# nerfstudio-project/nerfstudio

Hardware: AMD Instinct MI355X
Metric: training rays/sec (4096 rays x 48 samples per GPU) (higher is better)
Workload: dtype f32

## Files before the change

### nerfstudio_amd/csrc/density_mlp.hip

```cpp
#include "common.h"
#include "density_point.h"
#include "proposal_chain.h"

namespace nsamd {

constexpr int kMlpBlock = 256;
constexpr int kMaxBlocks = 768;
constexpr int kDensityActMax = 2048;

__host__ __device__ constexpr int density_partial_stride(int in_dim, int hidden) {
  return (hidden * in_dim + 2 * hidden + 1 + 3) & ~3;
}

template <int IN, int H>
__global__ __launch_bounds__(kMlpBlock) void density_mlp_fwd_kernel(const float* __restrict__ enc,
                                                                    const float* __restrict__ selector, int64_t M,
                                                                    nsamd_density_mlp mlp,
                                                                    float* __restrict__ density,
                                                                    float* __restrict__ pre_out) {
  const float* __restrict__ W0 = mlp.W0;
  const float* __restrict__ b0 = mlp.b0;
  const float* __restrict__ W1 = mlp.W1;
  for (int64_t p = (int64_t)blockIdx.x * kMlpBlock + threadIdx.x; p < M; p += (int64_t)gridDim.x * kMlpBlock) {
    float x[IN];
#pragma unroll
    for (int k = 0; k < IN; ++k) x[k] = enc[(int64_t)k * M + p];
    float out = mlp.b1[0];
    constexpr int JU = (H <= 16) ? H : 4;
#pragma unroll JU
    for (int j = 0; j < H; ++j) {
      float a = b0[j];
#pragma unroll
      for (int k = 0; k < IN; ++k) a = fmaf(W0[j * IN + k], x[k], a);
      out = fmaf(W1[j], fmaxf(a, 0.0f), out);
    }
    const float sel = selector ? selector[p] : 1.0f;
    if (pre_out) pre_out[p] = out;
    density[p] = mlp.average_init_density * expf(out) * sel;
  }
}

template <int LEVELS, int H>
__global__ __launch_bounds__(kMlpBlock) void density_field_fwd_kernel(nsamd_points P, int64_t M, int transform,
                                                                      nsamd_aabb box, const float2* __restrict__ table,
                                                                      nsamd_grid grid, nsamd_density_mlp mlp,
                                                                      float* __restrict__ enc_out,
                                                                      float* __restrict__ selector_out,
                                                                      float* __restrict__ density,
                                                                      float* __restrict__ pre_out) {
  const int64_t p = (int64_t)blockIdx.x * kMlpBlock + threadIdx.x;
  if (p >= M) return;
  float x, y, z;
  load_position(P, p, x, y, z);
  density_point<LEVELS, H>(x, y, z, p, M, transform, box, table, grid, mlp, enc_out, selector_out, density, pre_out);
// ... 179 lines not shown
    float* row = partials + (size_t)blockIdx.x * density_partial_stride(IN, H);
    for (int e = threadIdx.x; e < H * IN; e += kMlpBlock) row[e] = red[(e / IN) * 16 + (e % IN)];
    if (threadIdx.x < 2 * H + 1) row[H * IN + threadIdx.x] = accV;
    return;
  }
  for (int e = threadIdx.x; e < H * IN; e += kMlpBlock) unsafeAtomicAdd(dW0 + e, red[(e / IN) * 16 + (e % IN)]);
  if (threadIdx.x < H) unsafeAtomicAdd(db0 + threadIdx.x, accV);
  else if (threadIdx.x < 2 * H) unsafeAtomicAdd(dW1 + (threadIdx.x - H), accV);
  else if (threadIdx.x == 2 * H) unsafeAtomicAdd(db1, accV);
}

template <int IN, int H>
__global__ __launch_bounds__(kMlpBlock) void density_mlp_bwd_kernel(
    const float* __restrict__ enc, const float* __restrict__ selector, const float* __restrict__ pre,
    const float* __restrict__ ddensity, int64_t M, nsamd_density_mlp mlp, float* __restrict__ denc,
    float* __restrict__ dW0, float* __restrict__ db0, float* __restrict__ dW1, float* __restrict__ db1,
    float* __restrict__ partials, const uint32_t* __restrict__ gate, const uint8_t* __restrict__ ray_mask, int spr) {
  density_mlp_bwd_body<IN, H>(enc, selector, pre, ddensity, M, mlp, denc, dW0, db0, dW1, db1, partials, gate, ray_mask, spr,
                              (int)gridDim.x);
}

struct DensityBwdArgs {
  const float* enc;
  const float* selector;
  const float* pre;
  const float* ddensity;
  int64_t M;
  nsamd_density_mlp mlp;
  float* denc;
  float* dW0;
  float* db0;
  float* dW1;
  float* db1;
  float* partials;
  const uint32_t* gate;
  const uint8_t* ray_mask;
  int spr;
  int nblocks;
};

template <int IN, int H>
__global__ __launch_bounds__(kMlpBlock) void density_mlp_bwd_pair_kernel(DensityBwdArgs a, DensityBwdArgs b) {
  if (blockIdx.y == 0) {
    if ((int)blockIdx.x >= a.nblocks) return;
    density_mlp_bwd_body<IN, H>(a.enc, a.selector, a.pre, a.ddensity, a.M, a.mlp, a.denc, a.dW0, a.db0, a.dW1, a.db1,
                                a.partials, a.gate, a.ray_mask, a.spr, a.nblocks);
  } else {
    if ((int)blockIdx.x >= b.nblocks) return;
    density_mlp_bwd_body<IN, H>(b.enc, b.selector, b.pre, b.ddensity, b.M, b.mlp, b.denc, b.dW0, b.db0, b.dW1, b.db1,
                                b.partials, b.gate, b.ray_mask, b.spr, b.nblocks);
  }
}

constexpr int kDwGroups = 16;
__device__ __forceinline__ void density_dw_reduce_body(const float* __restrict__ partials, int rows, int stride, int n_w0,
                                                       int hidden, float* __restrict__ dW0, float* __restrict__ db0,
                                                       float* __restrict__ dW1, float* __restrict__ db1,
                                                       const uint32_t* __restrict__ gate) {
  if (gate != nullptr && __hip_atomic_load(gate, __ATOMIC_RELAXED, __HIP_MEMORY_SCOPE_AGENT) == 0u) return;
  __shared__ float part[kDwGroups][64];
  const int el = threadIdx.x & 63, grp = threadIdx.x >> 6;
  const int e = blockIdx.x * 64 + el;
  const int total = n_w0 + 2 * hidden + 1;
  float s = 0.f;
  if (e < total) {
    for (int b0i = grp; b0i < rows; b0i += kDwGroups * 16) {
      float v[16];
#pragma unroll
      for (int u = 0; u < 16; ++u) {
        const int b = b0i + u * kDwGroups;
        v[u] = partials[(size_t)(b < rows ? b : rows - 1) * stride + e];
      }
#pragma unroll
      for (int u = 0; u < 16; ++u) s += (b0i + u * kDwGroups < rows) ? v[u] : 0.0f;
    }
  }
  part[grp][el] = s;
  __syncthreads();
  if (grp == 0 && e < total) {
    float t = 0.f;
#pragma unroll
    for (int g2 = 0; g2 < kDwGroups; ++g2) t += part[g2][el];
    float* dst = e < n_w0 ? dW0 + e : (e < n_w0 + hidden ? db0 + (e - n_w0) : (e < n_w0 + 2 * hidden ? dW1 + (e - n_w0 - hidden) : db1));
    *dst += t;
  }
}

__global__ __launch_bounds__(64 * kDwGroups) void density_dw_reduce_kernel(const float* __restrict__ partials, int rows,
                                                                            int stride, int n_w0, int hidden,
                                                                            float* __restrict__ dW0,
                                                                            float* __restrict__ db0,
                                                                            float* __restrict__ dW1,
                                                                            float* __restrict__ db1,
                                                                            const uint32_t* __restrict__ gate) {
  density_dw_reduce_body(partials, rows, stride, n_w0, hidden, dW0, db0, dW1, db1, gate);
}

__global__ __launch_bounds__(64 * kDwGroups) void density_dw_reduce_pair_kernel(DensityBwdArgs a, DensityBwdArgs b, int stride,
                                                                                 int n_w0, int hidden) {
  if (blockIdx.y == 0) density_dw_reduce_body(a.partials, a.nblocks, stride, n_w0, hidden, a.dW0, a.db0, a.dW1, a.db1, a.gate);
  else density_dw_reduce_body(b.partials, b.nblocks, stride, n_w0, hidden, b.dW0, b.db0, b.dW1, b.db1, b.gate);
}

template <int IN, int H>
static int launch_fwd(const float* enc, const float* selector, int64_t M, nsamd_density_mlp mlp, float* density,
                      float* pre, hipStream_t stream) {
  const unsigned blocks = (unsigned)min((int64_t)8192, (M + kMlpBlock - 1) / kMlpBlock);
  density_mlp_fwd_kernel<IN, H><<<blocks, kMlpBlock, 0, stream>>>(enc, selector, M, mlp, density, pre);
  NSAMD_CHECK_LAUNCH();
  return NSAMD_OK;
}

template <int IN, int H>
static int launch_bwd(const float* enc, const float* selector, const float* pre, const float* ddensity, int64_t M,
                      nsamd_density_mlp mlp, float* denc, float* dW0, float* db0, float* dW1, float* db1,
                      float* workspace, int64_t workspace_floats, const uint32_t* gate, const uint8_t* ray_mask, int spr,
                      hipStream_t stream) {
  const unsigned blocks = (unsigned)min((int64_t)kMaxBlocks, (M + kMlpBlock - 1) / kMlpBlock);
  const size_t lds = sizeof(float) * ((size_t)(2 * H + IN + 1) * (kMlpBlock + 1) + 8 + (size_t)H * (((IN + 3) & ~3) + 2)) +
                     kDensityActMax;
  if (lds > 64 * 1024) {
    if (hipFuncSetAttribute(reinterpret_cast<const void*>(&density_mlp_bwd_kernel<IN, H>),
                            hipFuncAttributeMaxDynamicSharedMemorySize, (int)lds) != hipSuccess)
      return NSAMD_ERR_LAUNCH;
  }
  constexpr int stride = density_partial_stride(IN, H);
  float* partials = (workspace != nullptr && workspace_floats >= (int64_t)blocks * stride) ? workspace : nullptr;
  density_mlp_bwd_kernel<IN, H><<<blocks, kMlpBlock, lds, stream>>>(enc, selector, pre, ddensity, M, mlp, denc, dW0,
                                                                   db0, dW1, db1, partials, gate, ray_mask, spr);
  NSAMD_CHECK_LAUNCH();
  if (partials != nullptr) {
    const int total = H * IN + 2 * H + 1;
    density_dw_reduce_kernel<<<(total + 63) / 64, 64 * kDwGroups, 0, stream>>>(partials, (int)blocks, stride, H * IN, H,
                                                                             dW0, db0, dW1, db1, gate);
    NSAMD_CHECK_LAUNCH();
  }
  return NSAMD_OK;
}

template <int IN, int H>
static int launch_bwd_pair(const DensityBwdCall& a, const DensityBwdCall& b, hipStream_t stream) {
  const DensityBwdCall* c[2] = {&a, &b};
  const size_t lds = sizeof(float) * ((size_t)(2 * H + IN + 1) * (kMlpBlock + 1) + 8 + (size_t)H * (((IN + 3) & ~3) + 2)) +
                     kDensityActMax;
  if (lds > 64 * 1024) {
    if (hipFuncSetAttribute(reinterpret_cast<const void*>(&density_mlp_bwd_pair_kernel<IN, H>),
                            hipFuncAttributeMaxDynamicSharedMemorySize, (int)lds) != hipSuccess)
      return NSAMD_ERR_LAUNCH;
  }
  constexpr int stride = density_partial_stride(IN, H);
  DensityBwdArgs k[2];
  unsigned gx = 0;
  for (int i = 0; i < 2; ++i) {
    const unsigned blocks = (unsigned)min((int64_t)kMaxBlocks, (c[i]->M + kMlpBlock - 1) / kMlpBlock);
    if (c[i]->workspace == nullptr || c[i]->workspace_floats < (int64_t)blocks * stride) return NSAMD_ERR_UNSUPPORTED;
    k[i] = DensityBwdArgs{c[i]->enc, c[i]->selector, c[i]->pre, c[i]->ddensity, c[i]->M, c[i]->mlp, c[i]->denc, c[i]->dW0,
                          c[i]->db0, c[i]->dW1, c[i]->db1, c[i]->workspace, c[i]->gate, c[i]->ray_mask,
                          c[i]->ray_mask ? c[i]->spr : 1, (int)blocks};
    gx = blocks > gx ? blocks : gx;
  }
  if (a.workspace == b.workspace || a.dW0 == b.dW0) return NSAMD_ERR_UNSUPPORTED;
  density_mlp_bwd_pair_kernel<IN, H><<<dim3(gx, 2u), kMlpBlock, lds, stream>>>(k[0], k[1]);
  NSAMD_CHECK_LAUNCH();
  const int total = H * IN + 2 * H + 1;
  density_dw_reduce_pair_kernel<<<dim3((total + 63) / 64, 2u), 64 * kDwGroups, 0, stream>>>(k[0], k[1], stride, H * IN, H);
  NSAMD_CHECK_LAUNCH();
  return NSAMD_OK;
}

int density_bwd_launch_pair(const DensityBwdCall& a, const DensityBwdCall& b, hipStream_t stream) {
  if (a.mlp.in_dim != b.mlp.in_dim || a.mlp.hidden != b.mlp.hidden || a.M <= 0 || b.M <= 0) return NSAMD_ERR_UNSUPPORTED;
  if (a.mlp.in_dim == 10 && a.mlp.hidden == 16) return launch_bwd_pair<10, 16>(a, b, stream);
  if (a.mlp.in_dim == 16 && a.mlp.hidden == 16) return launch_bwd_pair<16, 16>(a, b, stream);
  if (a.mlp.in_dim == 10 && a.mlp.hidden == 64) return launch_bwd_pair<10, 64>(a, b, stream);
  if (a.mlp.in_dim == 16 && a.mlp.hidden == 64) return launch_bwd_pair<16, 64>(a, b, stream);
  return NSAMD_ERR_UNSUPPORTED;
}

}

using namespace nsamd;

#define NSAMD_DENSITY_DISPATCH(CALL)                                  \
  if (mlp.in_dim == 10 && mlp.hidden == 16) return CALL(10, 16);      \
  if (mlp.in_dim == 16 && mlp.hidden == 16) return CALL(16, 16);      \
  if (mlp.in_dim == 10 && mlp.hidden == 64) return CALL(10, 64);      \
  if (mlp.in_dim == 16 && mlp.hidden == 64) return CALL(16, 64);      \
  return NSAMD_ERR_UNSUPPORTED;

extern "C" int nsamd_density_mlp_fwd(const float* enc, const float* selector, int64_t M, nsamd_density_mlp mlp,
                                     float* density, float* pre, nsamd_stream_t stream) {
  NSAMD_REQUIRE(M >= 0);
  if (M == 0) return NSAMD_OK;
  NSAMD_REQUIRE(enc && density && mlp.W0 && mlp.b0 && mlp.W1 && mlp.b1);
#define CALL(IN, H) launch_fwd<IN, H>(enc, selector, M, mlp, density, pre, (hipStream_t)stream)
  NSAMD_DENSITY_DISPATCH(CALL)
#undef CALL
}

extern "C" int nsamd_density_field_fwd(nsamd_points pts, int64_t M, int transform, nsamd_aabb aabb, const float* table,
                                       nsamd_grid grid, nsamd_density_mlp mlp, float* enc, float* selector, float* density,
                                       float* pre, nsamd_stream_t stream) {
  NSAMD_REQUIRE(M >= 0);
  if (M == 0) return NSAMD_OK;
  NSAMD_REQUIRE(table && density && mlp.W0 && mlp.b0 && mlp.W1 && mlp.b1);
  NSAMD_REQUIRE(transform >= 0 && transform <= 2);
  if (pts.positions == nullptr) {
    NSAMD_REQUIRE(pts.origins && pts.directions && pts.t_bins && pts.samples_per_ray > 0 && M % pts.samples_per_ray == 0);
  }
  if (grid.log2_table_size < 1 || grid.log2_table_size > 28) return NSAMD_ERR_UNSUPPORTED;
  if (mlp.in_dim != 2 * grid.num_levels) return NSAMD_ERR_INVALID_ARG;
  const int64_t nb = (M + kMlpBlock - 1) / kMlpBlock;
  if (nb > 0x7fffffffLL) return NSAMD_ERR_UNSUPPORTED;
  const float2* t2 = reinterpret_cast<const float2*>(table);
#define NSAMD_DENSITY_FWD(L_, H_)                                                                                       \
  density_field_fwd_kernel<L_, H_><<<(unsigned)nb, kMlpBlock, 0, (hipStream_t)stream>>>(pts, M, transform, aabb, t2, grid, mlp, \
                                                                                      enc, selector, density, pre)
  if (grid.num_levels == 5 && mlp.hidden == 16) {
    NSAMD_DENSITY_FWD(5, 16);
  } else if (grid.num_levels == 8 && mlp.hidden == 16) {
    NSAMD_DENSITY_FWD(8, 16);
  } else if (grid.num_levels == 5 && mlp.hidden == 64) {
    NSAMD_DENSITY_FWD(5, 64);
  } else if (grid.num_levels == 8 && mlp.hidden == 64) {
    NSAMD_DENSITY_FWD(8, 64);
  } else {
    return NSAMD_ERR_UNSUPPORTED;
  }
// ... 35 lines not shown
```

### nerfstudio_amd/csrc/proposal_chain.h

```cpp
#pragma once

#include "common.h"

namespace nsamd {

struct WeightsBwdCall {
  const float* t_bins;
  const float* density;
  const float* dweights;
  int64_t num_rays;
  int32_t S;
  float* ddensity;
  uint32_t* gate;
  uint8_t* ray_mask;
};
int weights_bwd_launch_pair(const WeightsBwdCall& a, const WeightsBwdCall& b, hipStream_t stream);

struct DensityBwdCall {
  const float* enc;
  const float* selector;
  const float* pre;
  const float* ddensity;
  int64_t M;
  nsamd_density_mlp mlp;
  float* denc;
  float* dW0;
  float* db0;
  float* dW1;
  float* db1;
  float* workspace;
  int64_t workspace_floats;
  const uint32_t* gate;
  const uint8_t* ray_mask;
  int spr;
};
int density_bwd_launch_pair(const DensityBwdCall& a, const DensityBwdCall& b, hipStream_t stream);

}
```

### nerfstudio_amd/csrc/proposal_chain.hip

```cpp
#include "proposal_chain.h"
#include "scatter.h"

using namespace nsamd;

static int level_checks(const nsamd_proposal_level_bwd& l) {
  NSAMD_REQUIRE(l.num_rays > 0 && l.samples_per_ray > 0 && l.samples_per_ray <= 1024);
  NSAMD_REQUIRE(l.t_bins && l.density && l.dweights && l.ddensity && l.gate && l.ray_mask);
  NSAMD_REQUIRE(l.enc && l.pre && l.denc && l.dW0 && l.db0 && l.dW1 && l.db1 && l.mlp.W0 && l.mlp.b0 && l.mlp.W1 && l.mlp.b1);
  NSAMD_REQUIRE(l.origins && l.directions && l.table && l.dtable && l.scatter_workspace);
  NSAMD_REQUIRE(l.transform >= 0 && l.transform <= 2);
  NSAMD_REQUIRE(l.grid.num_levels > 0 && l.grid.num_levels <= NSAMD_MAX_LEVELS && 2 * l.grid.num_levels == l.mlp.in_dim);
  if (l.grid.log2_table_size < 1 || l.grid.log2_table_size > 28) return NSAMD_ERR_UNSUPPORTED;
  return NSAMD_OK;
}

static nsamd_points level_points(const nsamd_proposal_level_bwd& l) {
  nsamd_points p{};
  p.positions = nullptr;
  p.origins = l.origins;
  p.directions = l.directions;
  p.t_bins = l.t_bins;
  p.samples_per_ray = l.samples_per_ray;
  return p;
}

static int weights_single(const nsamd_proposal_level_bwd& l, nsamd_stream_t st) {
  return nsamd_weights_bwd_gate(l.t_bins, l.density, l.dweights, l.num_rays, l.samples_per_ray, l.ddensity, l.gate, l.ray_mask,
                                1, st);
}
static int density_single(const nsamd_proposal_level_bwd& l, nsamd_stream_t st) {
  return nsamd_density_mlp_bwd_gated(l.enc, l.selector, l.pre, l.ddensity, l.num_rays * l.samples_per_ray, l.mlp, l.denc, l.dW0,
                                     l.db0, l.dW1, l.db1, l.mlp_workspace, l.mlp_workspace_floats, l.gate, l.ray_mask,
                                     l.samples_per_ray, st);
}
static int scatter_single(const nsamd_proposal_level_bwd& l, nsamd_stream_t st) {
  const int64_t M = l.num_rays * l.samples_per_ray;
  return nsamd_hashgrid_encode_bwd_gated(level_points(l), M, l.transform, l.aabb, l.table, l.grid, l.denc, 1, M, l.dtable,
                                         l.scatter_workspace, l.scatter_workspace_floats, l.gate, l.ray_mask, st);
}

extern "C" int nsamd_proposal_levels_bwd(const nsamd_proposal_level_bwd* levels, int32_t num_levels, int32_t gates_precleared,
                                         nsamd_stream_t stream) {
  NSAMD_REQUIRE(num_levels >= 0 && (num_levels == 0 || levels != nullptr));
  hipStream_t st = (hipStream_t)stream;
  for (int i = 0; i < num_levels; ++i) {
    const int rc = level_checks(levels[i]);
    if (rc) return rc;
  }
  if (!gates_precleared) {
    for (int i = 0; i < num_levels; ++i)
      if (hipMemsetAsync(levels[i].gate, 0, sizeof(uint32_t), st) != hipSuccess) return NSAMD_ERR_LAUNCH;
  }
  for (int i = 0; i < num_levels; i += 2) {
    const nsamd_proposal_level_bwd& a = levels[i];
    if (i + 1 >= num_levels) {
      int rc = weights_single(a, stream);
      if (!rc) rc = density_single(a, stream);
      if (!rc) rc = scatter_single(a, stream);
      if (rc) return rc;
      break;
    }
    const nsamd_proposal_level_bwd& b = levels[i + 1];
    const int64_t Ma = a.num_rays * a.samples_per_ray, Mb = b.num_rays * b.samples_per_ray;
    int rc = weights_bwd_launch_pair(
        WeightsBwdCall{a.t_bins, a.density, a.dweights, a.num_rays, a.samples_per_ray, a.ddensity, a.gate, a.ray_mask},
        WeightsBwdCall{b.t_bins, b.density, b.dweights, b.num_rays, b.samples_per_ray, b.ddensity, b.gate, b.ray_mask}, st);
    if (rc == NSAMD_ERR_UNSUPPORTED) {
      rc = weights_single(a, stream);
      if (!rc) rc = weights_single(b, stream);
    }
    if (rc) return rc;
    rc = density_bwd_launch_pair(
        DensityBwdCall{a.enc, a.selector, a.pre, a.ddensity, Ma, a.mlp, a.denc, a.dW0, a.db0, a.dW1, a.db1, a.mlp_workspace,
                       a.mlp_workspace_floats, a.gate, a.ray_mask, a.samples_per_ray},
        DensityBwdCall{b.enc, b.selector, b.pre, b.ddensity, Mb, b.mlp, b.denc, b.dW0, b.db0, b.dW1, b.db1, b.mlp_workspace,
                       b.mlp_workspace_floats, b.gate, b.ray_mask, b.samples_per_ray},
        st);
    if (rc == NSAMD_ERR_UNSUPPORTED) {
      rc = density_single(a, stream);
      if (!rc) rc = density_single(b, stream);
    }
    if (rc) return rc;
    ScatterPlan pa = scatter_plan(a.grid, Ma, false), pb = scatter_plan(b.grid, Mb, false);
    rc = NSAMD_ERR_UNSUPPORTED;
    if (pa.ok && pb.ok && pa.total_words <= a.scatter_workspace_floats && pb.total_words <= b.scatter_workspace_floats) {
      rc = scatter_launch_pair(
          ScatterCall{level_points(a), Ma, a.transform, a.aabb, a.grid, a.denc, 1, Ma, a.dtable, a.scatter_workspace, pa, false,
                      a.gate, a.ray_mask},
          ScatterCall{level_points(b), Mb, b.transform, b.aabb, b.grid, b.denc, 1, Mb, b.dtable, b.scatter_workspace, pb, false,
                      b.gate, b.ray_mask},
          st);
    }
    if (rc == NSAMD_ERR_UNSUPPORTED) {
      rc = scatter_single(a, stream);
      if (!rc) rc = scatter_single(b, stream);
    }
    if (rc) return rc;
  }
  return NSAMD_OK;
}
```

### nerfstudio_amd/csrc/scatter.h

```cpp
#pragma once

#include "common.h"

namespace nsamd {

struct FixedScale {
  int k;
  bool empty;
  bool bad;
};

__device__ __forceinline__ FixedScale fixed_scale(uint32_t max_bits, int headroom) {
  FixedScale s;
  const int e_max = (int)((max_bits >> 23) & 0xffu);
  s.empty = e_max == 0;
  s.bad = e_max == 255;
  s.k = 188 - headroom - e_max;
  return s;
}

#ifndef NSAMD_FIXED_ROUND
#define NSAMD_FIXED_ROUND 0
#endif
__device__ __forceinline__ unsigned long long to_fixed(float v, int k) {
// ... 99 lines not shown
    float* a = t + 2 * (size_t)(rec.w & 0x3fffu);
    unsafeAtomicAdd(a, f0);
    unsafeAtomicAdd(a + 1, f1);
  }
  atomicAdd(hdr + kHdrEvtUnordered, 1u);
}

__device__ __forceinline__ void spill_append(const ScatterBufs& buf, uint32_t cap, uint32_t tile, const uint4& rec) {
  if (spill_list_append(buf.hdr, buf.spill_rec, buf.spill_tile, cap, tile, rec)) return;
  if (buf.direct_table != nullptr) {
    const uint32_t level = tile >> buf.log2_bins, bin = tile & ((1u << buf.log2_bins) - 1u);
    spill_direct(buf.direct_table + ((((size_t)level << buf.log2_table_size) + ((size_t)bin << buf.slice_log2)) << 1),
                 buf.hdr, rec);
  } else {
    atomicAdd(buf.hdr + kHdrEvtLost, 1u);
  }
}

struct PairHash {
  uint32_t ia, ib;
};

__device__ __forceinline__ PairHash pair_hash(const Cell& c, int q, uint32_t mask) {
  const uint32_t yz = ((uint32_t)((q & 1) ? c.hi[1] : c.lo[1]) * kPrimeY) ^ ((uint32_t)((q & 2) ? c.hi[2] : c.lo[2]) * kPrimeZ);
  return PairHash{((uint32_t)c.lo[0] ^ yz) & mask, ((uint32_t)c.hi[0] ^ yz) & mask};
}

#endif

struct ScatterPlan {
  bool ok;
  ScatterGeom geom;
  int64_t tiles;
  int64_t state_words;
  int64_t total_words;
};

ScatterPlan scatter_plan(const nsamd_grid& grid, int64_t M, bool max_spill);

ScatterPlan scatter_plan_producers(const nsamd_grid& grid, int64_t M, int workgroups, int seg_cap);

ScatterBufs scatter_bufs(float* workspace, const ScatterPlan& p);

struct ReduceRider;
bool scatter_apply_takes_rider(const ScatterPlan& plan);
int scatter_apply_launch(const nsamd_grid& grid, const ScatterPlan& plan, float* workspace, float* dtable, bool overwrite,
                         hipStream_t stream, const ReduceRider* rider = nullptr);

int scatter_launch(const nsamd_points& pts, int64_t M, int transform, const nsamd_aabb& aabb, const nsamd_grid& grid,
                   const float* denc, int64_t stride_p, int64_t stride_k, float* dtable, float* workspace,
                   const ScatterPlan& plan, bool overwrite, const uint32_t* gate, const uint8_t* ray_mask,
                   hipStream_t stream);

struct ScatterCall {
  nsamd_points pts;
  int64_t M;
  int transform;
  nsamd_aabb aabb;
  nsamd_grid grid;
  const float* denc;
  int64_t stride_p, stride_k;
  float* dtable;
  float* workspace;
  ScatterPlan plan;
  bool overwrite;
  const uint32_t* gate;
  const uint8_t* ray_mask;
};
int scatter_launch_pair(const ScatterCall& a, const ScatterCall& b, hipStream_t stream);

}
```

### nerfstudio_amd/csrc/scatter.hip

```cpp

#include <type_traits>

#include "field_reduce.h"
#include "scatter.h"

NSAMD_PROBE_DEFINE(scatter)

namespace nsamd {

__device__ __forceinline__ bool gate_is_clear(const uint32_t* gate) {
  return gate != nullptr && __hip_atomic_load(gate, __ATOMIC_RELAXED, __HIP_MEMORY_SCOPE_AGENT) == 0u;
}

constexpr int kRunLen = 4;
constexpr int kRunThreads = 256;
constexpr int kMaxLog2Bins = 10;

template <int kThreads, int kPts, int kLevels>
__global__ __launch_bounds__(kThreads) void scatter_route_fine_kernel(
    nsamd_points P, int64_t M, int transform, nsamd_aabb box, nsamd_grid grid, const float* __restrict__ denc,
    int64_t stride_p, int64_t stride_k, ScatterGeom G, LevelList levels, ScatterBufs buf,
    const uint32_t* __restrict__ gate, const uint8_t* __restrict__ ray_mask) {
  static_assert(kPts * kLevels * 4 <= 32, "overflow mask is 32 bits");
  if (gate_is_clear(gate)) return;
  extern __shared__ __attribute__((aligned(16))) uint32_t lds_u[];
  const int B = 1 << G.log2_bins;
  uint32_t* cnt = lds_u;
  uint32_t* cnt2 = cnt + kLevels * B;
  uint32_t* base = cnt2 + kLevels * B;
  uint32_t* lmax = base + kLevels * B;
  PROBE_STAMP(0, 0);
  for (int t = threadIdx.x; t < 2 * kLevels * B; t += kThreads) cnt[t] = 0u;
  if (threadIdx.x < kLevels) lmax[threadIdx.x] = 0u;
  const int first = blockIdx.y * kLevels;
  int lvl[kLevels];
#pragma unroll
  for (int i = 0; i < kLevels; ++i) lvl[i] = first + i < levels.count ? (int)levels.level[first + i] : -1;
  float g0[kPts][kLevels], g1[kPts][kLevels];
  float x[kPts], y[kPts], z[kPts];
  bool inside[kPts];
  uint8_t mask_raw[kPts];
  int64_t pcl[kPts];
#pragma unroll
  for (int j = 0; j < kPts; ++j) {
    const int64_t p = ((int64_t)blockIdx.x * kPts + j) * kThreads + threadIdx.x;
    inside[j] = p < M;
    pcl[j] = inside[j] ? p : M - 1;
    mask_raw[j] = ray_mask != nullptr ? ray_mask[pcl[j] / P.samples_per_ray] : (uint8_t)1;
  }
  if (ray_mask != nullptr) {
    bool marked = false;
#pragma unroll
    for (int j = 0; j < kPts; ++j) marked = marked || (inside[j] && mask_raw[j] != 0);
    if (!__syncthreads_or(marked)) {
      for (int t = threadIdx.x; t < kLevels * B; t += kThreads) {
// ... 490 lines not shown
  __syncthreads();
  PROBE_STAMP(0, 15);
  float4* out = reinterpret_cast<float4*>(
      dtable + ((((size_t)level << grid.log2_table_size) + ((size_t)bin << G.slice_log2)) << 1));
  const uint4* a4 = reinterpret_cast<const uint4*>(acc);
  const float nan = __uint_as_float(0x7fc00000u);
  for (int i = threadIdx.x; i < entries / 2; i += blockDim.x) {
    const uint4 e0 = a4[2 * i], e1 = a4[2 * i + 1];
    float4 v;
    if (fs.bad) {
      v = make_float4(nan, nan, nan, nan);
    } else {
      v.x = from_fixed(((unsigned long long)e0.y << 32) | e0.x, fs.k);
      v.y = from_fixed(((unsigned long long)e0.w << 32) | e0.z, fs.k);
      v.z = from_fixed(((unsigned long long)e1.y << 32) | e1.x, fs.k);
      v.w = from_fixed(((unsigned long long)e1.w << 32) | e1.z, fs.k);
    }
    if (overwrite) {
      out[i] = v;
    } else if ((e0.x | e0.y | e0.z | e0.w | e1.x | e1.y | e1.z | e1.w) != 0u || fs.bad) {
      float4 o = out[i];
      o.x += v.x; o.y += v.y; o.z += v.z; o.w += v.w;
      out[i] = o;
    }
  }
  PROBE_STAMP(0, 16);
}

template <bool kRider>
__global__ void scatter_apply_kernel(nsamd_grid grid, ScatterGeom G, ScatterBufs buf, float* __restrict__ dtable,
                                     int overwrite, const uint32_t* __restrict__ gate, ReduceRider rider) {
  scatter_apply_body<kRider>(grid, G, buf, dtable, overwrite, gate, rider);
}

struct ApplyCall {
  nsamd_grid grid;
  ScatterGeom G;
  ScatterBufs buf;
  float* dtable;
  int overwrite;
  const uint32_t* gate;
};

__global__ void scatter_apply_pair_kernel(ApplyCall a, ApplyCall b) {
  if (blockIdx.z == 0) {
    if (blockIdx.x >= (1u << a.G.log2_bins) || (int)blockIdx.y >= a.G.num_levels) return;
    scatter_apply_body<false>(a.grid, a.G, a.buf, a.dtable, a.overwrite, a.gate, ReduceRider{});
  } else {
    if (blockIdx.x >= (1u << b.G.log2_bins) || (int)blockIdx.y >= b.G.num_levels) return;
    scatter_apply_body<false>(b.grid, b.G, b.buf, b.dtable, b.overwrite, b.gate, ReduceRider{});
  }
}

__device__ __forceinline__ void scatter_finish_body(const nsamd_grid& grid, const ScatterGeom& G, const ScatterBufs& buf,
                                                    float* __restrict__ dtable, const uint32_t* __restrict__ gate) {
  if (gate_is_clear(gate)) return;
  const uint32_t total = buf.hdr[kHdrSpillCount];
  const uint32_t n = min(total, G.spill_cap);
  for (uint32_t e = kSpillFold + blockIdx.x * blockDim.x + threadIdx.x; e < n; e += gridDim.x * blockDim.x) {
    const uint4 r = buf.spill_rec[e];
    const uint32_t tile = buf.spill_tile[e];
    const uint32_t level = tile >> G.log2_bins, bin = tile & ((1u << G.log2_bins) - 1u);
    float* t = dtable + ((((size_t)level << grid.log2_table_size) + ((size_t)bin << G.slice_log2)) << 1);
    const float f0 = __uint_as_float(r.x), f1 = __uint_as_float(r.y);
    if (r.w & 0x80000000u) {
      const float wx = __uint_as_float(r.z), omx = 1.0f - wx;
      float* a = t + 2 * (size_t)(r.w & 0x3fffu);
      float* b = t + 2 * (size_t)((r.w >> 14) & 0x3fffu);
      unsafeAtomicAdd(a, f0 * omx);
      unsafeAtomicAdd(a + 1, f1 * omx);
      unsafeAtomicAdd(b, f0 * wx);
      unsafeAtomicAdd(b + 1, f1 * wx);
    } else {
      float* a = t + 2 * (size_t)(r.w & 0x3fffu);
      unsafeAtomicAdd(a, f0);
      unsafeAtomicAdd(a + 1, f1);
    }
  }
  __syncthreads();
  if (threadIdx.x == 0 && atomicAdd(buf.hdr + kHdrTicket, 1u) == gridDim.x - 1) {
    for (int l = 0; l < NSAMD_MAX_LEVELS; ++l) buf.hdr[l] = 0u;
    if (total) {
      buf.hdr[kHdrEvtSpill] += total;
      if (n > kSpillFold) buf.hdr[kHdrEvtUnordered] += n - kSpillFold;
    }
    buf.hdr[kHdrSpillCount] = 0u;
    buf.hdr[kHdrTicket] = 0u;
  }
}

__global__ void scatter_finish_kernel(nsamd_grid grid, ScatterGeom G, ScatterBufs buf, float* __restrict__ dtable,
                                      const uint32_t* __restrict__ gate) {
  scatter_finish_body(grid, G, buf, dtable, gate);
}

__global__ void scatter_finish_pair_kernel(ApplyCall a, ApplyCall b) {
  if (blockIdx.z == 0) scatter_finish_body(a.grid, a.G, a.buf, a.dtable, a.gate);
  else scatter_finish_body(b.grid, b.G, b.buf, b.dtable, b.gate);
}

static unsigned apply_threads(int slice_log2);

constexpr int kFineThreads = 1024, kFineLevels = 4;
constexpr int kScatterTargetTiles = 512;

constexpr int kSliceLog2Max = 13;

ScatterPlan scatter_plan(const nsamd_grid& grid, int64_t M, bool max_spill) {
  ScatterPlan p{};
  if (M <= 0 || grid.num_levels <= 0 || grid.num_levels > NSAMD_MAX_LEVELS) return p;
  int bits = 0;
  while ((grid.num_levels << bits) < kScatterTargetTiles) ++bits;
  int sl = grid.log2_table_size - bits;
  float res_max = 0.0f;
  for (int l = 0; l < grid.num_levels; ++l) res_max = grid.scalings[l] > res_max ? grid.scalings[l] : res_max;
  int sl_pair = 1;
  while ((1 << sl_pair) < (int)res_max + 2 && sl_pair < kSliceLog2Max) ++sl_pair;
  sl = sl < sl_pair ? sl_pair : sl;
  sl = sl > kSliceLog2Max ? kSliceLog2Max : (sl < 8 ? 8 : sl);
  if (sl > grid.log2_table_size) sl = grid.log2_table_size;
  const int log2_bins = grid.log2_table_size - sl;
  if (log2_bins > kMaxLog2Bins) return p;
  ScatterGeom& g = p.geom;
  g.slice_log2 = sl;
  g.log2_bins = log2_bins;
  g.num_levels = grid.num_levels;
  g.block_points = (uint32_t)kFineThreads;
  const int64_t bins = (int64_t)1 << log2_bins;
  const int64_t segs = (M + g.block_points - 1) / g.block_points;
  int64_t C = 2 * ((4 * (int64_t)g.block_points + bins - 1) / bins);
  C = (C + 3) & ~(int64_t)3;
  if (C < 16) C = 16;
  const int64_t expect = (4 * M + bins - 1) / bins;
  int64_t Qn = segs * C + expect / 2 + 64;
  if (Qn < 2 * expect + expect / 2 + 64) Qn = 2 * expect + expect / 2 + 64;
  Qn = (Qn + 3) & ~(int64_t)3;
  int64_t Qs = segs * C + 6 * expect + 64;
  if (Qs < 8 * expect + 64) Qs = 8 * expect + 64;
  Qs = (Qs + 3) & ~(int64_t)3;
  p.tiles = bins * grid.num_levels;
  int64_t total = 0, Qmax = 0;
  for (int l = 0; l < grid.num_levels; ++l) {
    const double lattice = ((double)grid.scalings[l] + 1.0) * ((double)grid.scalings[l] + 1.0) * ((double)grid.scalings[l] + 1.0);
    const int64_t Ql = lattice * 2.0 <= (double)((int64_t)1 << grid.log2_table_size) ? Qs : Qn;
    if (total >= 0x7fffffffLL) return p;
    g.level_off[l] = (uint32_t)total;
    g.level_cap[l] = (uint32_t)Ql;
    total += bins * Ql;
    Qmax = Ql > Qmax ? Ql : Qmax;
// ... 59 lines not shown
  g.seg_cap = (uint32_t)C;
  const int64_t spill = 4 * M * grid.num_levels + 64;
  if (spill >= 0x7fffffffLL) return p;
  g.spill_cap = (uint32_t)spill;
  g.headroom = 0;
  g.coarse_mask = 0u;
  const int64_t cursor_words = (p.tiles + 3) & ~(int64_t)3;
  const int64_t count_words = (p.tiles * segs + 3) & ~(int64_t)3;
  p.state_words = kHdrWords + cursor_words;
  p.total_words = kHdrWords + cursor_words + count_words + 4 * total + 4 * spill + ((spill + 3) & ~(int64_t)3);
  p.ok = true;
  return p;
}

static int apply_lds_attribute() {
  static bool attr_done[64] = {};
  int dev = 0;
  if (hipGetDevice(&dev) != hipSuccess) return NSAMD_ERR_NO_DEVICE;
  if (dev < 0 || dev >= 64 || !attr_done[dev]) {
    if (hipFuncSetAttribute(reinterpret_cast<const void*>(&scatter_apply_kernel<false>),
                            hipFuncAttributeMaxDynamicSharedMemorySize, (int)(16u << kSliceLog2Max)) != hipSuccess ||
        hipFuncSetAttribute(reinterpret_cast<const void*>(&scatter_apply_kernel<true>),
                            hipFuncAttributeMaxDynamicSharedMemorySize, (int)(16u << kSliceLog2Max)) != hipSuccess ||
        hipFuncSetAttribute(reinterpret_cast<const void*>(&scatter_apply_pair_kernel),
                            hipFuncAttributeMaxDynamicSharedMemorySize, (int)(16u << kSliceLog2Max)) != hipSuccess)
      return NSAMD_ERR_LAUNCH;
    if (dev >= 0 && dev < 64) attr_done[dev] = true;
  }
  return NSAMD_OK;
}

int scatter_apply_launch(const nsamd_grid& grid, const ScatterPlan& plan, float* workspace, float* dtable, bool overwrite,
                         hipStream_t st, const ReduceRider* rider) {
  ScatterGeom G = plan.geom;
  ScatterBufs buf = scatter_bufs(workspace, plan);
  buf.log2_table_size = grid.log2_table_size;
  if (!overwrite) buf.direct_table = dtable;
  int rc = apply_lds_attribute();
  if (rc) return rc;
  const unsigned threads = apply_threads(G.slice_log2);
  ReduceRider rd{};
  unsigned extra_rows = 0u;
  if (rider != nullptr && rider->blocks > 0) {
    if (threads != (unsigned)kReduceThreads) return NSAMD_ERR_UNSUPPORTED;
    rd = *rider;
    extra_rows = ((unsigned)rd.blocks + (1u << G.log2_bins) - 1u) >> G.log2_bins;
  }
  dim3 g2(1u << G.log2_bins, (unsigned)grid.num_levels + extra_rows);
  if (extra_rows != 0u)
    scatter_apply_kernel<true><<<g2, threads, (size_t)16 << G.slice_log2, st>>>(grid, G, buf, dtable, overwrite ? 1 : 0, nullptr, rd);
  else
    scatter_apply_kernel<false><<<g2, threads, (size_t)16 << G.slice_log2, st>>>(grid, G, buf, dtable, overwrite ? 1 : 0, nullptr, rd);
  NSAMD_CHECK_LAUNCH();
  scatter_finish_kernel<<<32, 256, 0, st>>>(grid, G, buf, dtable, nullptr);
  NSAMD_CHECK_LAUNCH();
  return NSAMD_OK;
}

static unsigned apply_threads(int slice_log2) {
  return slice_log2 > 11 ? 1024u : (slice_log2 > 9 ? 512u : 256u);
}

bool scatter_apply_takes_rider(const ScatterPlan& plan) { return apply_threads(plan.geom.slice_log2) == 1024u; }

ScatterBufs scatter_bufs(float* workspace, const ScatterPlan& p) {
  ScatterBufs b;
  uint32_t* w = reinterpret_cast<uint32_t*>(workspace);
  b.hdr = w;
  b.dyn_cursor = w + kHdrWords;
  const int64_t cursor_words = (p.tiles + 3) & ~(int64_t)3;
  b.counts = b.dyn_cursor + cursor_words;
  const int64_t count_words = (p.tiles * (int64_t)p.geom.segs + 3) & ~(int64_t)3;
  b.queues = reinterpret_cast<uint4*>(b.counts + count_words);
  b.spill_rec = b.queues + (size_t)p.geom.queue_records;
  b.spill_tile = reinterpret_cast<uint32_t*>(b.spill_rec + p.geom.spill_cap);
  b.direct_table = nullptr;
  b.log2_table_size = 0;
  b.log2_bins = p.geom.log2_bins;
  b.slice_log2 = p.geom.slice_log2;
  return b;
}

static void classify_levels(const nsamd_points& pts, const nsamd_grid& grid, ScatterGeom& G, LevelList& coarse,
                            LevelList& fine) {
  float coarse_below = 0.0f;
  if (pts.positions == nullptr && pts.samples_per_ray >= 96)
    coarse_below = pts.samples_per_ray >= 192 ? (float)pts.samples_per_ray : 1e30f;
  for (int l = 0; l < grid.num_levels; ++l) {
    if (grid.scalings[l] < coarse_below) {
      G.coarse_mask |= 1u << l;
      coarse.level[coarse.count++] = (int8_t)l;
    } else {
      fine.level[fine.count++] = (int8_t)l;
    }
  }
}

constexpr int kRunLevels = 2;

int scatter_launch(const nsamd_points& pts, int64_t M, int transform, const nsamd_aabb& aabb, const nsamd_grid& grid,
                   const float* denc, int64_t stride_p, int64_t stride_k, float* dtable, float* workspace,
                   const ScatterPlan& plan, bool overwrite, const uint32_t* gate, const uint8_t* ray_mask, hipStream_t st) {
  if (gate != nullptr && overwrite) return NSAMD_ERR_INVALID_ARG;
  if (ray_mask != nullptr && (gate == nullptr || pts.positions != nullptr)) return NSAMD_ERR_INVALID_ARG;
  ScatterGeom G = plan.geom;
  ScatterBufs buf = scatter_bufs(workspace, plan);
  buf.log2_table_size = grid.log2_table_size;
  if (!overwrite) buf.direct_table = dtable;
  LevelList coarse{}, fine{};
  classify_levels(pts, grid, G, coarse, fine);
  {
    const int rc = apply_lds_attribute();
    if (rc) return rc;
  }
  if (fine.count > 0) {
    const size_t lds = sizeof(uint32_t) * (3 * (size_t)kFineLevels * ((size_t)1 << G.log2_bins) + kFineLevels);
    dim3 g1(G.segs, (unsigned)((fine.count + kFineLevels - 1) / kFineLevels));
    scatter_route_fine_kernel<kFineThreads, 1, kFineLevels><<<g1, kFineThreads, lds, st>>>(
        pts, M, transform, aabb, grid, denc, stride_p, stride_k, G, fine, buf, gate, ray_mask);
    NSAMD_CHECK_LAUNCH();
  }
  if (coarse.count > 0) {
    constexpr int kL = kRunLevels;
    const int64_t per_block = (int64_t)kRunThreads * kRunLen;
    const size_t lds = sizeof(uint32_t) * (3 * (size_t)kL * ((size_t)1 << G.log2_bins) + kL);
    dim3 g1((unsigned)((M + per_block - 1) / per_block), (unsigned)((coarse.count + kL - 1) / kL));
    scatter_route_runs_kernel<kL><<<g1, kRunThreads, lds, st>>>(pts, M, transform, aabb, grid, denc, stride_p, stride_k, G,
                                                              coarse, buf, gate, ray_mask);
    NSAMD_CHECK_LAUNCH();
  }
  const unsigned threads = apply_threads(G.slice_log2);
  dim3 g2(1u << G.log2_bins, (unsigned)grid.num_levels);
  scatter_apply_kernel<false><<<g2, threads, (size_t)16 << G.slice_log2, st>>>(grid, G, buf, dtable, overwrite ? 1 : 0, gate,
                                                                               ReduceRider{});
  NSAMD_CHECK_LAUNCH();
  scatter_finish_kernel<<<32, 256, 0, st>>>(grid, G, buf, dtable, gate);
  NSAMD_CHECK_LAUNCH();
  return NSAMD_OK;
}

int scatter_launch_pair(const ScatterCall& a, const ScatterCall& b, hipStream_t st) {
  const ScatterCall* c[2] = {&a, &b};
  ScatterGeom G[2];
  ScatterBufs buf[2];
  LevelList coarse[2], fine[2];
  for (int i = 0; i < 2; ++i) {
    if (c[i]->gate != nullptr && c[i]->overwrite) return NSAMD_ERR_INVALID_ARG;
    if (c[i]->ray_mask != nullptr && (c[i]->gate == nullptr || c[i]->pts.positions != nullptr)) return NSAMD_ERR_INVALID_ARG;
    if (!c[i]->plan.ok || c[i]->M <= 0) return NSAMD_ERR_UNSUPPORTED;
    G[i] = c[i]->plan.geom;
    buf[i] = scatter_bufs(c[i]->workspace, c[i]->plan);
    buf[i].log2_table_size = c[i]->grid.log2_table_size;
    if (!c[i]->overwrite) buf[i].direct_table = c[i]->dtable;
    coarse[i] = LevelList{};
    fine[i] = LevelList{};
    classify_levels(c[i]->pts, c[i]->grid, G[i], coarse[i], fine[i]);
    if (fine[i].count != 0 || coarse[i].count == 0) return NSAMD_ERR_UNSUPPORTED;
  }
  if (a.workspace == b.workspace || a.dtable == b.dtable) return NSAMD_ERR_UNSUPPORTED;
  const unsigned threads = apply_threads(G[0].slice_log2);
  if (threads != apply_threads(G[1].slice_log2)) return NSAMD_ERR_UNSUPPORTED;
  {
    const int rc = apply_lds_attribute();
    if (rc) return rc;
  }
  constexpr int kL = kRunLevels;
  const int64_t per_block = (int64_t)kRunThreads * kRunLen;
  RunsCall rc[2];
  size_t run_lds = 0;
  unsigned gx = 0, gy = 0;
  for (int i = 0; i < 2; ++i) {
    rc[i] = RunsCall{c[i]->pts, c[i]->M, c[i]->transform, c[i]->aabb, c[i]->grid, c[i]->denc, c[i]->stride_p, c[i]->stride_k,
                     G[i], coarse[i], buf[i], c[i]->gate, c[i]->ray_mask,
                     (uint32_t)((c[i]->M + per_block - 1) / per_block), (uint32_t)((coarse[i].count + kL - 1) / kL)};
    const size_t l = sizeof(uint32_t) * (3 * (size_t)kL * ((size_t)1 << G[i].log2_bins) + kL);
    run_lds = l > run_lds ? l : run_lds;
    gx = rc[i].grid_x > gx ? rc[i].grid_x : gx;
    gy = rc[i].grid_y > gy ? rc[i].grid_y : gy;
  }
  scatter_route_runs_pair_kernel<kL><<<dim3(gx, gy, 2u), kRunThreads, run_lds, st>>>(rc[0], rc[1]);
  NSAMD_CHECK_LAUNCH();
  ApplyCall ac[2];
  unsigned bins = 0, levels = 0;
  size_t lds = 0;
  for (int i = 0; i < 2; ++i) {
    ac[i] = ApplyCall{c[i]->grid, G[i], buf[i], c[i]->dtable, c[i]->overwrite ? 1 : 0, c[i]->gate};
    bins = (1u << G[i].log2_bins) > bins ? (1u << G[i].log2_bins) : bins;
    levels = (unsigned)c[i]->grid.num_levels > levels ? (unsigned)c[i]->grid.num_levels : levels;
    const size_t l = (size_t)16 << G[i].slice_log2;
    lds = l > lds ? l : lds;
  }
  scatter_apply_pair_kernel<<<dim3(bins, levels, 2u), threads, lds, st>>>(ac[0], ac[1]);
  NSAMD_CHECK_LAUNCH();
  scatter_finish_pair_kernel<<<dim3(32u, 1u, 2u), 256, 0, st>>>(ac[0], ac[1]);
  NSAMD_CHECK_LAUNCH();
  return NSAMD_OK;
}

}
```

Baseline: 6.656 million.

## Defer density weight-gradient reduce into scatter finish pair kernel launch

The paired density-MLP weight-gradient reduction is no longer launched right after the backward kernel. It is deferred and carried as a rider into the scatter finish pair kernel, where extra blocks past the first 32 run the reduce body. This removes one kernel launch per proposal step and lets the reduce overlap the scatter's spill finishing. In exchange, the finish kernel now launches with 1024-thread blocks, so the scatter finish loop strides by a fixed block count. A fallback path still launches the reduce separately when the paired scatter is unsupported.

```diff
diff --git a/nerfstudio_amd/csrc/density_mlp.hip b/nerfstudio_amd/csrc/density_mlp.hip
--- a/nerfstudio_amd/csrc/density_mlp.hip
+++ b/nerfstudio_amd/csrc/density_mlp.hip
@@ -1,5 +1,6 @@
 #include "common.h"
 #include "density_point.h"
+#include "density_reduce.h"
 #include "proposal_chain.h"
 
 namespace nsamd {
@@ -285,54 +286,19 @@
   }
 }
 
-constexpr int kDwGroups = 16;
-__device__ __forceinline__ void density_dw_reduce_body(const float* __restrict__ partials, int rows, int stride, int n_w0,
-                                                       int hidden, float* __restrict__ dW0, float* __restrict__ db0,
-                                                       float* __restrict__ dW1, float* __restrict__ db1,
-                                                       const uint32_t* __restrict__ gate) {
-  if (gate != nullptr && __hip_atomic_load(gate, __ATOMIC_RELAXED, __HIP_MEMORY_SCOPE_AGENT) == 0u) return;
-  __shared__ float part[kDwGroups][64];
-  const int el = threadIdx.x & 63, grp = threadIdx.x >> 6;
-  const int e = blockIdx.x * 64 + el;
-  const int total = n_w0 + 2 * hidden + 1;
-  float s = 0.f;
-  if (e < total) {
-    for (int b0i = grp; b0i < rows; b0i += kDwGroups * 16) {
-      float v[16];
-#pragma unroll
-      for (int u = 0; u < 16; ++u) {
-        const int b = b0i + u * kDwGroups;
-        v[u] = partials[(size_t)(b < rows ? b : rows - 1) * stride + e];
-      }
-#pragma unroll
-      for (int u = 0; u < 16; ++u) s += (b0i + u * kDwGroups < rows) ? v[u] : 0.0f;
-    }
-  }
-  part[grp][el] = s;
-  __syncthreads();
-  if (grp == 0 && e < total) {
-    float t = 0.f;
-#pragma unroll
-    for (int g2 = 0; g2 < kDwGroups; ++g2) t += part[g2][el];
-    float* dst = e < n_w0 ? dW0 + e : (e < n_w0 + hidden ? db0 + (e - n_w0) : (e < n_w0 + 2 * hidden ? dW1 + (e - n_w0 - hidden) : db1));
-    *dst += t;
-  }
-}
-
-__global__ __launch_bounds__(64 * kDwGroups) void density_dw_reduce_kernel(const float* __restrict__ partials, int rows,
-                                                                            int stride, int n_w0, int hidden,
-                                                                            float* __restrict__ dW0,
-                                                                            float* __restrict__ db0,
-                                                                            float* __restrict__ dW1,
-                                                                            float* __restrict__ db1,
-                                                                            const uint32_t* __restrict__ gate) {
-  density_dw_reduce_body(partials, rows, stride, n_w0, hidden, dW0, db0, dW1, db1, gate);
-}
-
-__global__ __launch_bounds__(64 * kDwGroups) void density_dw_reduce_pair_kernel(DensityBwdArgs a, DensityBwdArgs b, int stride,
-                                                                                 int n_w0, int hidden) {
-  if (blockIdx.y == 0) density_dw_reduce_body(a.partials, a.nblocks, stride, n_w0, hidden, a.dW0, a.db0, a.dW1, a.db1, a.gate);
-  else density_dw_reduce_body(b.partials, b.nblocks, stride, n_w0, hidden, b.dW0, b.db0, b.dW1, b.db1, b.gate);
+__global__ __launch_bounds__(kDensityReduceThreads) void density_dw_reduce_kernel(const float* __restrict__ partials, int rows,
+                                                                                int stride, int n_w0, int hidden,
+                                                                                float* __restrict__ dW0,
+                                                                                float* __restrict__ db0,
+                                                                                float* __restrict__ dW1,
+                                                                                float* __restrict__ db1,
+                                                                                const uint32_t* __restrict__ gate) {
+  density_dw_reduce_body((int)blockIdx.x, partials, rows, stride, n_w0, hidden, dW0, db0, dW1, db1, gate);
+}
+
+__global__ __launch_bounds__(kDensityReduceThreads) void density_dw_reduce_pair_kernel(DensityReduceRider r) {
+  const DensityReduceCall& c = blockIdx.y == 0 ? r.call[0] : r.call[1];
+  density_dw_reduce_body((int)blockIdx.x, c.partials, c.rows, r.stride, r.n_w0, r.hidden, c.dW0, c.db0, c.dW1, c.db1, c.gate);
 }
 
 template <int IN, int H>
@@ -364,7 +330,7 @@
   NSAMD_CHECK_LAUNCH();
   if (partials != nullptr) {
     const int total = H * IN + 2 * H + 1;
-    density_dw_reduce_kernel<<<(total + 63) / 64, 64 * kDwGroups, 0, stream>>>(partials, (int)blocks, stride, H * IN, H,
+    density_dw_reduce_kernel<<<(total + 63) / 64, kDensityReduceThreads, 0, stream>>>(partials, (int)blocks, stride, H * IN, H,
                                                                              dW0, db0, dW1, db1, gate);
     NSAMD_CHECK_LAUNCH();
   }
@@ -372,7 +338,8 @@
 }
 
 template <int IN, int H>
-static int launch_bwd_pair(const DensityBwdCall& a, const DensityBwdCall& b, hipStream_t stream) {
+static int launch_bwd_pair(const DensityBwdCall& a, const DensityBwdCall& b, DensityReduceRider* deferred,
+                           hipStream_t stream) {
   const DensityBwdCall* c[2] = {&a, &b};
   const size_t lds = sizeof(float) * ((size_t)(2 * H + IN + 1) * (kMlpBlock + 1) + 8 + (size_t)H * (((IN + 3) & ~3) + 2)) +
                      kDensityActMax;
@@ -395,18 +362,31 @@
   if (a.workspace == b.workspace || a.dW0 == b.dW0) return NSAMD_ERR_UNSUPPORTED;
   density_mlp_bwd_pair_kernel<IN, H><<<dim3(gx, 2u), kMlpBlock, lds, stream>>>(k[0], k[1]);
   NSAMD_CHECK_LAUNCH();
-  const int total = H * IN + 2 * H + 1;
-  density_dw_reduce_pair_kernel<<<dim3((total + 63) / 64, 2u), 64 * kDwGroups, 0, stream>>>(k[0], k[1], stride, H * IN, H);
+  DensityReduceRider r{};
+  for (int i = 0; i < 2; ++i) r.call[i] = DensityReduceCall{k[i].partials, k[i].nblocks, k[i].dW0, k[i].db0, k[i].dW1, k[i].db1, k[i].gate};
+  r.stride = stride, r.n_w0 = H * IN, r.hidden = H;
+  r.blocks = (H * IN + 2 * H + 1 + 63) / 64;
+  if (deferred != nullptr) {
+    *deferred = r;
+    return NSAMD_OK;
+  }
+  return density_reduce_launch_pair(r, stream);
+}
+
+int density_reduce_launch_pair(const DensityReduceRider& r, hipStream_t stream) {
+  if (r.blocks <= 0) return NSAMD_OK;
+  density_dw_reduce_pair_kernel<<<dim3((unsigned)r.blocks, 2u), kDensityReduceThreads, 0, stream>>>(r);
   NSAMD_CHECK_LAUNCH();
   return NSAMD_OK;
 }
 
-int density_bwd_launch_pair(const DensityBwdCall& a, const DensityBwdCall& b, hipStream_t stream) {
+int density_bwd_launch_pair(const DensityBwdCall& a, const DensityBwdCall& b, DensityReduceRider* deferred,
+                            hipStream_t stream) {
   if (a.mlp.in_dim != b.mlp.in_dim || a.mlp.hidden != b.mlp.hidden || a.M <= 0 || b.M <= 0) return NSAMD_ERR_UNSUPPORTED;
-  if (a.mlp.in_dim == 10 && a.mlp.hidden == 16) return launch_bwd_pair<10, 16>(a, b, stream);
-  if (a.mlp.in_dim == 16 && a.mlp.hidden == 16) return launch_bwd_pair<16, 16>(a, b, stream);
-  if (a.mlp.in_dim == 10 && a.mlp.hidden == 64) return launch_bwd_pair<10, 64>(a, b, stream);
-  if (a.mlp.in_dim == 16 && a.mlp.hidden == 64) return launch_bwd_pair<16, 64>(a, b, stream);
+  if (a.mlp.in_dim == 10 && a.mlp.hidden == 16) return launch_bwd_pair<10, 16>(a, b, deferred, stream);
+  if (a.mlp.in_dim == 16 && a.mlp.hidden == 16) return launch_bwd_pair<16, 16>(a, b, deferred, stream);
+  if (a.mlp.in_dim == 10 && a.mlp.hidden == 64) return launch_bwd_pair<10, 64>(a, b, deferred, stream);
+  if (a.mlp.in_dim == 16 && a.mlp.hidden == 64) return launch_bwd_pair<16, 64>(a, b, deferred, stream);
   return NSAMD_ERR_UNSUPPORTED;
 }
 
diff --git a/nerfstudio_amd/csrc/density_reduce.h b/nerfstudio_amd/csrc/density_reduce.h
--- /dev/null
+++ b/nerfstudio_amd/csrc/density_reduce.h
@@ -0,0 +1,59 @@
+#pragma once
+
+#include "common.h"
+
+namespace nsamd {
+
+constexpr int kDwGroups = 16;
+constexpr int kDensityReduceThreads = 64 * kDwGroups;
+
+__device__ __forceinline__ void density_dw_reduce_body(int block, const float* __restrict__ partials, int rows, int stride,
+                                                       int n_w0, int hidden, float* __restrict__ dW0,
+                                                       float* __restrict__ db0, float* __restrict__ dW1,
+                                                       float* __restrict__ db1, const uint32_t* __restrict__ gate) {
+  if (gate != nullptr && __hip_atomic_load(gate, __ATOMIC_RELAXED, __HIP_MEMORY_SCOPE_AGENT) == 0u) return;
+  __shared__ float part[kDwGroups][64];
+  const int el = threadIdx.x & 63, grp = threadIdx.x >> 6;
+  const int e = block * 64 + el;
+  const int total = n_w0 + 2 * hidden + 1;
+  float s = 0.f;
+  if (e < total) {
+    for (int b0i = grp; b0i < rows; b0i += kDwGroups * 16) {
+      float v[16];
+#pragma unroll
+      for (int u = 0; u < 16; ++u) {
+        const int b = b0i + u * kDwGroups;
+        v[u] = partials[(size_t)(b < rows ? b : rows - 1) * stride + e];
+      }
+#pragma unroll
+      for (int u = 0; u < 16; ++u) s += (b0i + u * kDwGroups < rows) ? v[u] : 0.0f;
+    }
+  }
+  part[grp][el] = s;
+  __syncthreads();
+  if (grp == 0 && e < total) {
+    float t = 0.f;
+#pragma unroll
+    for (int g2 = 0; g2 < kDwGroups; ++g2) t += part[g2][el];
+    float* dst = e < n_w0 ? dW0 + e : (e < n_w0 + hidden ? db0 + (e - n_w0) : (e < n_w0 + 2 * hidden ? dW1 + (e - n_w0 - hidden) : db1));
+    *dst += t;
+  }
+}
+
+struct DensityReduceCall {
+  const float* partials;
+  int rows;
+  float* dW0;
+  float* db0;
+  float* dW1;
+  float* db1;
+  const uint32_t* gate;
+};
+
+struct DensityReduceRider {
+  DensityReduceCall call[2];
+  int stride, n_w0, hidden;
+  int blocks;
+};
+
+}
diff --git a/nerfstudio_amd/csrc/proposal_chain.h b/nerfstudio_amd/csrc/proposal_chain.h
--- a/nerfstudio_amd/csrc/proposal_chain.h
+++ b/nerfstudio_amd/csrc/proposal_chain.h
@@ -34,6 +34,8 @@
   const uint8_t* ray_mask;
   int spr;
 };
-int density_bwd_launch_pair(const DensityBwdCall& a, const DensityBwdCall& b, hipStream_t stream);
+struct DensityReduceRider;
+int density_bwd_launch_pair(const DensityBwdCall& a, const DensityBwdCall& b, DensityReduceRider* deferred, hipStream_t stream);
+int density_reduce_launch_pair(const DensityReduceRider& rider, hipStream_t stream);
 
 }
diff --git a/nerfstudio_amd/csrc/proposal_chain.hip b/nerfstudio_amd/csrc/proposal_chain.hip
--- a/nerfstudio_amd/csrc/proposal_chain.hip
+++ b/nerfstudio_amd/csrc/proposal_chain.hip
@@ -1,4 +1,5 @@
 #include "proposal_chain.h"
+#include "density_reduce.h"
 #include "scatter.h"
 
 using namespace nsamd;
@@ -70,13 +71,15 @@
       if (!rc) rc = weights_single(b, stream);
     }
     if (rc) return rc;
+    DensityReduceRider reduce{};
     rc = density_bwd_launch_pair(
         DensityBwdCall{a.enc, a.selector, a.pre, a.ddensity, Ma, a.mlp, a.denc, a.dW0, a.db0, a.dW1, a.db1, a.mlp_workspace,
                        a.mlp_workspace_floats, a.gate, a.ray_mask, a.samples_per_ray},
         DensityBwdCall{b.enc, b.selector, b.pre, b.ddensity, Mb, b.mlp, b.denc, b.dW0, b.db0, b.dW1, b.db1, b.mlp_workspace,
                        b.mlp_workspace_floats, b.gate, b.ray_mask, b.samples_per_ray},
-        st);
+        &reduce, st);
     if (rc == NSAMD_ERR_UNSUPPORTED) {
+      reduce.blocks = 0;
       rc = density_single(a, stream);
       if (!rc) rc = density_single(b, stream);
     }
@@ -89,10 +92,11 @@
                       a.gate, a.ray_mask},
           ScatterCall{level_points(b), Mb, b.transform, b.aabb, b.grid, b.denc, 1, Mb, b.dtable, b.scatter_workspace, pb, false,
                       b.gate, b.ray_mask},
-          st);
+          st, reduce.blocks > 0 ? &reduce : nullptr);
     }
     if (rc == NSAMD_ERR_UNSUPPORTED) {
-      rc = scatter_single(a, stream);
+      rc = density_reduce_launch_pair(reduce, st);
+      if (!rc) rc = scatter_single(a, stream);
       if (!rc) rc = scatter_single(b, stream);
     }
     if (rc) return rc;
diff --git a/nerfstudio_amd/csrc/scatter.h b/nerfstudio_amd/csrc/scatter.h
--- a/nerfstudio_amd/csrc/scatter.h
+++ b/nerfstudio_amd/csrc/scatter.h
@@ -175,6 +175,7 @@
                    const ScatterPlan& plan, bool overwrite, const uint32_t* gate, const uint8_t* ray_mask,
                    hipStream_t stream);
 
+struct DensityReduceRider;
 struct ScatterCall {
   nsamd_points pts;
   int64_t M;
@@ -190,6 +191,7 @@
   const uint32_t* gate;
   const uint8_t* ray_mask;
 };
-int scatter_launch_pair(const ScatterCall& a, const ScatterCall& b, hipStream_t stream);
+int scatter_launch_pair(const ScatterCall& a, const ScatterCall& b, hipStream_t stream,
+                        const DensityReduceRider* reduce = nullptr);
 
 }
diff --git a/nerfstudio_amd/csrc/scatter.hip b/nerfstudio_amd/csrc/scatter.hip
--- a/nerfstudio_amd/csrc/scatter.hip
+++ b/nerfstudio_amd/csrc/scatter.hip
@@ -1,6 +1,7 @@
 
 #include <type_traits>
 
+#include "density_reduce.h"
 #include "field_reduce.h"
 #include "scatter.h"
 
@@ -597,12 +598,13 @@
   }
 }
 
+constexpr unsigned kFinishBlocks = 32;
 __device__ __forceinline__ void scatter_finish_body(const nsamd_grid& grid, const ScatterGeom& G, const ScatterBufs& buf,
                                                     float* __restrict__ dtable, const uint32_t* __restrict__ gate) {
   if (gate_is_clear(gate)) return;
   const uint32_t total = buf.hdr[kHdrSpillCount];
   const uint32_t n = min(total, G.spill_cap);
-  for (uint32_t e = kSpillFold + blockIdx.x * blockDim.x + threadIdx.x; e < n; e += gridDim.x * blockDim.x) {
+  for (uint32_t e = kSpillFold + blockIdx.x * blockDim.x + threadIdx.x; e < n; e += kFinishBlocks * blockDim.x) {
     const uint4 r = buf.spill_rec[e];
     const uint32_t tile = buf.spill_tile[e];
     const uint32_t level = tile >> G.log2_bins, bin = tile & ((1u << G.log2_bins) - 1u);
@@ -623,7 +625,7 @@
     }
   }
   __syncthreads();
-  if (threadIdx.x == 0 && atomicAdd(buf.hdr + kHdrTicket, 1u) == gridDim.x - 1) {
+  if (threadIdx.x == 0 && atomicAdd(buf.hdr + kHdrTicket, 1u) == kFinishBlocks - 1) {
     for (int l = 0; l < NSAMD_MAX_LEVELS; ++l) buf.hdr[l] = 0u;
     if (total) {
       buf.hdr[kHdrEvtSpill] += total;
@@ -639,7 +641,13 @@
   scatter_finish_body(grid, G, buf, dtable, gate);
 }
 
-__global__ void scatter_finish_pair_kernel(ApplyCall a, ApplyCall b) {
+__global__ void scatter_finish_pair_kernel(ApplyCall a, ApplyCall b, DensityReduceRider rider) {
+  if (blockIdx.x >= kFinishBlocks) {
+    const DensityReduceCall& c = blockIdx.z == 0 ? rider.call[0] : rider.call[1];
+    density_dw_reduce_body((int)(blockIdx.x - kFinishBlocks), c.partials, c.rows, rider.stride, rider.n_w0, rider.hidden, c.dW0,
+                           c.db0, c.dW1, c.db1, c.gate);
+    return;
+  }
   if (blockIdx.z == 0) scatter_finish_body(a.grid, a.G, a.buf, a.dtable, a.gate);
   else scatter_finish_body(b.grid, b.G, b.buf, b.dtable, b.gate);
 }
@@ -805,7 +813,7 @@
   else
     scatter_apply_kernel<false><<<g2, threads, (size_t)16 << G.slice_log2, st>>>(grid, G, buf, dtable, overwrite ? 1 : 0, nullptr, rd);
   NSAMD_CHECK_LAUNCH();
-  scatter_finish_kernel<<<32, 256, 0, st>>>(grid, G, buf, dtable, nullptr);
+  scatter_finish_kernel<<<kFinishBlocks, 256, 0, st>>>(grid, G, buf, dtable, nullptr);
   NSAMD_CHECK_LAUNCH();
   return NSAMD_OK;
 }
@@ -887,12 +895,12 @@
   scatter_apply_kernel<false><<<g2, threads, (size_t)16 << G.slice_log2, st>>>(grid, G, buf, dtable, overwrite ? 1 : 0, gate,
                                                                                ReduceRider{});
   NSAMD_CHECK_LAUNCH();
-  scatter_finish_kernel<<<32, 256, 0, st>>>(grid, G, buf, dtable, gate);
+  scatter_finish_kernel<<<kFinishBlocks, 256, 0, st>>>(grid, G, buf, dtable, gate);
   NSAMD_CHECK_LAUNCH();
   return NSAMD_OK;
 }
 
-int scatter_launch_pair(const ScatterCall& a, const ScatterCall& b, hipStream_t st) {
+int scatter_launch_pair(const ScatterCall& a, const ScatterCall& b, hipStream_t st, const DensityReduceRider* reduce) {
   const ScatterCall* c[2] = {&a, &b};
   ScatterGeom G[2];
   ScatterBufs buf[2];
@@ -945,7 +953,12 @@
   }
   scatter_apply_pair_kernel<<<dim3(bins, levels, 2u), threads, lds, st>>>(ac[0], ac[1]);
   NSAMD_CHECK_LAUNCH();
-  scatter_finish_pair_kernel<<<dim3(32u, 1u, 2u), 256, 0, st>>>(ac[0], ac[1]);
+  if (reduce != nullptr && reduce->blocks > 0) {
+    scatter_finish_pair_kernel<<<dim3(kFinishBlocks + (unsigned)reduce->blocks, 1u, 2u), kDensityReduceThreads, 0, st>>>(
+        ac[0], ac[1], *reduce);
+  } else {
+    scatter_finish_pair_kernel<<<dim3(kFinishBlocks, 1u, 2u), 256, 0, st>>>(ac[0], ac[1], DensityReduceRider{});
+  }
   NSAMD_CHECK_LAUNCH();
   return NSAMD_OK;
 }
```

Result: no change. 6.708 million (median of 6 runs) (+0.8%).
